# mfigura/Resilient-consensus-based-MARL

Measured on AMD Instinct MI355X. Metric: agent-steps/sec (whole RPBCAC training loop; + consensus-updates/sec), higher is better.
Workload: dtype f32 (matrix-core operands as 2 x f16 pieces: each fp32 operand to <= 1 ulp; the 20-unit layers run 3 of the 4 piece products)

## Files before the change

### include/rcmarl.h

```cpp
#ifndef RCMARL_H
#define RCMARL_H

#ifdef __cplusplus
extern "C" {
#endif

#define RCMARL_OK 0
#define RCMARL_ERR_ARG 1
#define RCMARL_ERR_LAUNCH 2
#define RCMARL_ERR_UNSUPPORTED 3

int rcmarl_abi_version(void);
int rcmarl_mb_job_layout(int what);
int rcmarl_fit_partial_size(int hid);
int rcmarl_actor_partial_size(int hid, int n_actions);
int rcmarl_rows_per_chunk(void);

int rcmarl_consensus_params(const float* msg, float* theta, const int* nbr, const int* coop, int S, int N,
                            int ldp, int P_hid, int d, int H, float* lo_dbg, float* hi_dbg, void* stream);
int rcmarl_consensus_params_circulant_supported(int N, int d, int H);
int rcmarl_consensus_params_circulant(const float* msg, float* theta, const int* coop, int S, int N, int ldp, int P_hid,
                                      int d, int H, float* lo_dbg, float* hi_dbg, void* stream);

typedef struct rcmarl_ragged_class {
// ... 15 lines not shown
                                float* adam_v, const int* mask, int S, int N, int B, int in_dim, int hid,
                                int ldp, int ldb, float alpha, float one_m_b1, float one_m_b2, float eps, void* stream);

int rcmarl_mid_fit(float* a1t, const float* theta, const float* y, float* partials, int S, int N, int B, int in_dim,
                   int hid, int ldp, int ldb, void* stream);
int rcmarl_lattice_f16_mode(void);
int rcmarl_lattice_set_f16_mode(int mode);
int rcmarl_lattice_forget(const void* buf);
int rcmarl_lattice_encode(const float* x, long x_seed_stride, const float* alpha, int S, int B, int in_dim, void* kp,
                          int kp_rt, int kp_kt, void* ktp, int ktp_rt, int ktp_kt, int* flag, void* stream);
int rcmarl_w1_split(const float* theta, const float* alpha, void* wp, int S, int N, int in_dim, int hid, int ldp,
                    int wp_rt, int wp_kt, void* stream);
int rcmarl_lattice_pack_dz(const float* dz, void* dzp, int S, int N, int B, int hid, int ldb, int dzp_rt, int dzp_kt,
                           void* stream);
int rcmarl_lattice_pack_dz_rowsum(const float* dz, void* dzp, float* sums, int sums_ld, int sums_off, int S, int N, int B, int hid,
                                  int ldb, int dzp_rt, int dzp_kt, void* stream);
int rcmarl_layer1_forward_lattice(const void* kp, int kp_rt, int kp_kt, const void* wp, int wp_rt, int wp_kt,
                                  const float* theta, float* a1t, int S, int N, int B, int in_dim, int hid, int ldp,
                                  int ldb, void* stream);
int rcmarl_layer1_backward_sgd_lattice(const void* ktp, int ktp_rt, int ktp_kt, const void* dzp, int dzp_rt, int dzp_kt,
                                       const float* alpha, float* theta, const int* mask, int S, int N, int B,
                                       int in_dim, int hid, int ldp, float lr, void* wp_out, int wp_rt, int wp_kt,
                                       void* stream);
int rcmarl_mid_fit_lattice(const float* a1t, const float* theta, const float* y, float* partials, void* dzp, int dzp_rt,
                           int dzp_kt, int S, int N, int B, int in_dim, int hid, int ldp, int ldb, int* ovf_flags, void* stream);


int rcmarl_shuffle_perms(const void* seeds, const int* calls, int n, int epochs, int B, int* perm, int S, void* stream);

int rcmarl_small_sgd(const float* partials, float* theta, const int* mask, float* loss_out, int S, int N,
                     int B, int in_dim, int hid, int ldp, float lr, void* stream);
int rcmarl_mid_value(const float* a1t, const float* theta, const float* r_applied, float gamma, float* out, int S,
                     int N, int B, int in_dim, int hid, int ldp, int ldb, void* stream);
int rcmarl_mid_value_f32(const float* a1t, const float* theta, const float* r_applied, float gamma, float* out, int S,
                         int N, int B, int in_dim, int hid, int ldp, int ldb, void* stream);

int rcmarl_consensus_head(const float* a1t, const float* theta, const float* msg, const int* nbr,
                          const int* coop, float* partials, float* agg_out, int S, int N, int B, int in_dim,
                          int hid, int ldp, int ldb, int d, int H, void* stream);
int rcmarl_consensus_head_ragged(const float* a1t, const float* theta, const float* msg, const int* nbr_off,
                                 const int* nbr_idx, const int* order, const rcmarl_ragged_class* classes, int n_classes,
                                 float* partials, float* agg_out, int S, int N, int B, int in_dim, int hid, int ldp, int ldb,
                                 void* stream);
int rcmarl_projection_residual(const float* a1t, const float* theta, const float* agg, const int* coop,
                               float* partials, int S, int N, int B, int in_dim, int hid, int ldp, int ldb,
                               void* stream);
// ... 167 lines not shown
```

### resilient-consensus-based-marl_amd/capi.py

```python
import ctypes as C
import os

c_f32p = C.c_void_p
c_i32p = C.c_void_p
c_u8p = C.c_void_p


class MbJob(C.Structure):
    _fields_ = [("x", C.c_void_p), ("x_seed_stride", C.c_long), ("theta", C.c_void_p), ("agents", C.c_void_p), ("n_adv", C.c_int),
                ("in_dim", C.c_int), ("ldp", C.c_int), ("reserved_", C.c_int), ("y", C.c_void_p), ("perm", C.c_void_p),
                ("loss_out", C.c_void_p), ("ovf_flags", C.c_void_p)]


class RaggedClass(C.Structure):
    _fields_ = [("d", C.c_int), ("H", C.c_int), ("first", C.c_int), ("count", C.c_int)]


c_f64p = C.c_void_p
c_stream = C.c_void_p

c_long = C.c_long
c_int = C.c_int
c_float = C.c_float

# ... 17 lines not shown
    "rcmarl_consensus_params_circulant": [c_f32p, c_f32p, c_u8p, c_int, c_int, c_int, c_int, c_int, c_int, c_f32p, c_f32p,
                                          c_stream],
    "rcmarl_ragged_class_layout": [c_int],
    "rcmarl_consensus_params_ragged": [c_f32p, c_f32p, c_i32p, c_i32p, c_i32p, C.c_void_p, c_int, c_int, c_int, c_int, c_int,
                                       c_f32p, c_f32p, c_stream],
    "rcmarl_consensus_head_ragged": [c_f32p, c_f32p, c_f32p, c_i32p, c_i32p, c_i32p, C.c_void_p, c_int, c_f32p, c_f32p, c_int,
                                     c_int, c_int, c_int, c_int, c_int, c_int, c_stream],
    "rcmarl_layer1_forward": [c_f32p, c_long, c_f32p, c_f32p, c_int, c_int, c_int, c_int, c_int, c_int, c_int,
                              c_stream],
    "rcmarl_layer1_backward_sgd": [c_f32p, c_long, c_f32p, c_f32p, c_u8p, c_int, c_int, c_int, c_int, c_int, c_int,
                                   c_int, c_float, c_stream],
    "rcmarl_layer1_backward_adam": [c_f32p, c_long, c_f32p, c_f32p, c_f32p, c_f32p, c_u8p, c_int, c_int, c_int, c_int,
                                    c_int, c_int, c_int, c_float, c_float, c_float, c_float, c_stream],
    "rcmarl_mid_fit": [c_f32p, c_f32p, c_f32p, c_f32p, c_int, c_int, c_int, c_int, c_int, c_int, c_int, c_stream],
    "rcmarl_lattice_encode": [c_f32p, c_long, c_f32p, c_int, c_int, c_int, c_u8p, c_int, c_int, c_u8p, c_int, c_int,
                              c_i32p, c_stream],
    "rcmarl_w1_split": [c_f32p, c_f32p, c_u8p, c_int, c_int, c_int, c_int, c_int, c_int, c_int, c_stream],
    "rcmarl_lattice_pack_dz": [c_f32p, c_u8p, c_int, c_int, c_int, c_int, c_int, c_int, c_int, c_stream],
    "rcmarl_lattice_pack_dz_rowsum": [c_f32p, c_u8p, c_f32p, c_int, c_int, c_int, c_int, c_int, c_int, c_int, c_int, c_int, c_stream],
    "rcmarl_layer1_forward_lattice": [c_u8p, c_int, c_int, c_u8p, c_int, c_int, c_f32p, c_f32p, c_int, c_int, c_int,
                                      c_int, c_int, c_int, c_int, c_stream],
    "rcmarl_layer1_backward_sgd_lattice": [c_u8p, c_int, c_int, c_u8p, c_int, c_int, c_f32p, c_f32p, c_u8p, c_int,
                                           c_int, c_int, c_int, c_int, c_int, c_float, c_u8p, c_int, c_int, c_stream],
    "rcmarl_mid_fit_lattice": [c_f32p, c_f32p, c_f32p, c_f32p, c_u8p, c_int, c_int, c_int, c_int, c_int, c_int, c_int,
                               c_int, c_int, c_i32p, c_stream],
    "rcmarl_shuffle_perms": [C.c_void_p, c_i32p, c_int, c_int, c_int, c_i32p, c_int, c_stream],
    "rcmarl_small_sgd": [c_f32p, c_f32p, c_u8p, c_f32p, c_int, c_int, c_int, c_int, c_int, c_int, c_float, c_stream],
    "rcmarl_mid_value": [c_f32p, c_f32p, c_f32p, c_float, c_f32p, c_int, c_int, c_int, c_int, c_int, c_int, c_int,
                         c_stream],
    "rcmarl_mid_value_f32": [c_f32p, c_f32p, c_f32p, c_float, c_f32p, c_int, c_int, c_int, c_int, c_int, c_int, c_int,
                             c_stream],
    "rcmarl_consensus_head": [c_f32p, c_f32p, c_f32p, c_i32p, c_u8p, c_f32p, c_f32p, c_int, c_int, c_int, c_int, c_int,
                              c_int, c_int, c_int, c_int, c_stream],
    "rcmarl_head_apply": [c_f32p, c_f32p, c_u8p, c_int, c_int, c_int, c_int, c_int, c_int, c_stream],
    "rcmarl_mid_actor": [c_f32p, c_f32p, c_f32p, c_f32p, c_f32p, c_int, c_int, c_int, c_int, c_int, c_int, c_int,
                         c_int, c_stream],
    "rcmarl_small_adam": [c_f32p, c_f32p, c_f32p, c_f32p, c_u8p, c_f32p, c_int, c_int, c_int, c_int, c_int, c_int,
                          c_int, c_float, c_float, c_float, c_float, c_stream],
    "rcmarl_team_reward": [c_f32p, c_long, c_u8p, c_int, c_f32p, c_int, c_int, c_int, c_int, c_stream],
    "rcmarl_projection_residual": [c_f32p, c_f32p, c_f32p, c_i32p, c_f32p, c_int, c_int, c_int, c_int, c_int, c_int,
                                   c_int, c_stream],
    "rcmarl_minibatch_fit": [c_f32p, c_long, c_f32p, c_i32p, c_int, c_f32p, c_i32p, c_int, c_int, c_int, c_int, c_int,
                             c_int, c_int, c_int, c_int, c_float, c_f32p, c_i32p, c_stream],
    "rcmarl_minibatch_actor": [c_f32p, c_long, c_f32p, c_f32p, c_f32p, c_i32p, c_int, c_f32p, c_f32p, c_i32p, c_int,
                               c_int, c_int, c_int, c_int, c_int, c_int, c_int, c_int, c_int, C.c_double, C.c_double,
                               C.c_double, C.c_double, c_int, c_f32p, c_stream],
# ... 58 lines not shown
    "rcmarl_policy_probs_wide": [c_f32p, c_f32p, c_f32p, c_int, c_int, c_int, c_int, c_int, c_int, c_stream],
    "rcmarl_rollout_step_wide": [c_f32p, c_i32p, c_i32p, c_f32p, C.c_void_p, c_int, c_int, c_f64p, c_f32p, c_f32p, c_f32p,
                                 c_f32p, c_f32p, c_long, c_long, c_i32p, c_f32p, c_f64p, C.c_double, c_int, c_int, c_float,
                                 c_int, c_int, c_int, c_int, c_int, c_i32p, c_stream],
    "rcmarl_rollout_wide_supported": [c_int],
    "rcmarl_policy_probs_episodes_wide": [c_f32p, c_f32p, c_f32p, c_int, c_int, c_int, c_int, c_int, c_int, c_int, c_stream],
    "rcmarl_rollout_step_episodes_wide": [c_f32p, c_i32p, c_i32p, c_f32p, C.c_void_p, c_int, c_int, c_f64p, c_f32p, c_f32p,
                                          c_f32p, c_f32p, c_f32p, c_long, c_long, c_int, c_i32p, c_f32p, c_f64p, C.c_double,
                                          c_int, c_int, c_float, c_int, c_int, c_int, c_int, c_int, c_int, c_int, c_stream],
    "rcmarl_dense_backward_adam": [c_f32p, c_long, c_long, c_int, c_int, c_f32p, c_f32p, c_f32p, c_f32p, c_int, c_i32p, c_int,
                                   c_int, c_int, c_int, c_int, c_int, c_int, c_float, c_float, c_float, c_float, c_stream],
    "rcmarl_wide_actor_head": [c_f32p, c_f32p, c_f32p, c_f32p, c_int, c_f32p, c_f32p, c_int, c_int, c_int, c_int, c_int, c_int,
                               c_int, c_int, c_stream],
    "rcmarl_wide_actor_small_adam": [c_f32p, c_f32p, c_f32p, c_f32p, c_f32p, c_f32p, c_f32p, c_i32p, c_f32p, c_int, c_int, c_int,
                                     c_int, c_int, c_int, c_int, c_int, c_float, c_float, c_float, c_float, c_stream],
    "rcmarl_copy3d": [c_f32p, c_long, c_long, c_f32p, c_long, c_long, c_int, c_int, c_int, c_i32p, c_stream],
}
UNCHECKED = {"rcmarl_abi_version", "rcmarl_mb_job_layout", "rcmarl_ragged_class_layout", "rcmarl_lattice_forget", "rcmarl_fit_partial_size", "rcmarl_lattice_set_f16_mode",  "rcmarl_actor_partial_size", "rcmarl_rows_per_chunk", "rcmarl_lattice_f16_mode",
             "rcmarl_wide_grad_size", "rcmarl_wide_rows_per_chunk", "rcmarl_wide_f16_mode", "rcmarl_wide_set_f16_mode",
             "rcmarl_consensus_params_circulant_supported", "rcmarl_pk_supported", "rcmarl_pk_parts",
             "rcmarl_rollout_wide_supported", "rcmarl_minibatch_fit_wide_supported",
             "rcmarl_minibatch_fit_wide2_supported"}

ERRORS = {1: "RCMARL_ERR_ARG (bad argument)", 2: "RCMARL_ERR_LAUNCH (HIP launch failed)",
          3: "RCMARL_ERR_UNSUPPORTED (shape outside the compiled kernels)"}


class RcmarlError(RuntimeError):
    pass


def _preload_hip_runtime():
    import torch
    cand = os.path.join(os.path.dirname(torch.__file__), "lib", "libamdhip64.so")
    try:
        C.CDLL(cand if os.path.exists(cand) else "libamdhip64.so.7", mode=C.RTLD_GLOBAL)
    except OSError as e:
        raise RcmarlError("cannot load the HIP runtime (libamdhip64): %s" % e)


class CLib:

    def __init__(self, path, needs_hip=True):
        if not os.path.exists(path):
            raise RcmarlError(
                "rcmarl HIP library not found at %s -- build it with `python -m rcmarl_amd.build` "
                "(hipcc --offload-arch=gfx950). There is no CPU fallback." % path)
        self.path = path
        if needs_hip:
            _preload_hip_runtime()
        self._dll = C.CDLL(path)
        for name, argtypes in SIGNATURES.items():
            fn = getattr(self._dll, name)
            fn.argtypes = argtypes
            fn.restype = C.c_int
            setattr(self, name, fn if name in UNCHECKED else self._checked(name, fn))

    @staticmethod
    def _checked(name, fn):
        def call(*args):
            rc = fn(*args)
            if rc != 0:
                raise RcmarlError("%s failed: %s" % (name, ERRORS.get(rc, rc)))
            return 0
        call.__name__ = name
        return call


_lib = None


def load():
    global _lib
    if _lib is None:
        from . import build
        _lib = CLib(build.lib_path())
    return _lib
```

### resilient-consensus-based-marl_amd/csrc/lattice_gemm.hip

```cpp
#include "rcmarl_lattice.h"
#include "rcmarl_lat_mainloop.h"
#include <type_traits>
#include <stdlib.h>

namespace {

__device__ __forceinline__ unsigned pack2(unsigned lo, unsigned hi) { return (lo & 0xffffu) | (hi << 16); }

__global__ __launch_bounds__(256) void k_lattice_encode(const float* __restrict__ x, long x_seed_stride,
                                                        const float* __restrict__ alpha, int B, int in_dim,
                                                        unsigned char* __restrict__ kp, int kp_rt, int kp_kt,
                                                        unsigned char* __restrict__ ktp, int ktp_rt, int ktp_kt,
                                                        int* __restrict__ flag, int kp_f16, int ktp_f16) {
  __shared__ unsigned short tileB[32][128 + 2], tileH[32][128 + 2];
  const int s = blockIdx.z, b0 = blockIdx.y * 32, c0 = blockIdx.x * 128;
  const int t = threadIdx.x;
  {
    const int cl = t & 127, c = c0 + cl;
    const float al = c < in_dim ? alpha[c] : 1.f;
    bool bad = false;
#pragma unroll 4
    for (int i = 0; i < 16; ++i) {
      const int bl = (t >> 7) + 2 * i, b = b0 + bl;
      float kq = 0.f;
// ... 272 lines not shown
    for (int nt = 0; nt < NT; ++nt) {
      const int n = bn * C::BN + wn * 32 * NT + 32 * nt + (lane & 31);
      if (n < B) {
        const unsigned lane_byte = ((unsigned)(4 * half) * (unsigned)ldb + (unsigned)n) * 4u;
#pragma unroll
        for (int mt = 0; mt < MT; ++mt) {
          const int m0 = bm * C::BM + wm * 32 * MT + 32 * mt;
          unsigned char* __restrict__ rowbase = reinterpret_cast<unsigned char*>(a1t_s + (long)m0 * ldb);
#pragma unroll
          for (int r = 0; r < 16; ++r) {
            const int dr = (r & 3) + 8 * (r >> 2);
            const float z = F16 ? fmaf(acc[mt][nt][r], RC_F16_W_UNSCALE, bv[mt][r]) : acc[mt][nt][r] + bv[mt][r];
            const float o = fmaxf(z, RC_LEAK * z);
            float* __restrict__ dst = reinterpret_cast<float*>(rowbase + (long)dr * ldb * 4 + lane_byte);
            if (FULL || m0 + dr + 4 * half < ncols) RC_NT_STORE(dst, o);
          }
        }
      }
    }
  };
  if (full_m) store_tile(std::true_type{}); else store_tile(std::false_type{});
}

template <bool W8, bool DZ16, bool WP16, bool M128 = false>
__global__ RC_LAT_OCC(W8 ? 512 : 256, W8 ? 4 : 2)
void k_lat_backward_sgd(const unsigned char* __restrict__ ktp, int ktp_rt, int ktp_kt, const unsigned char* __restrict__ dzp,
                        int dzp_rt, int dzp_kt, const float* __restrict__ alpha, float* __restrict__ theta,
                        const int* __restrict__ mask, int S, int N, int B, int in_dim, int ldp, float lr, int mtiles, int ntiles,
                        unsigned char* __restrict__ wp_out, int wp_rt, int wp_kt, int hid) {
  static_assert(!(W8 && M128), "the 128-row tile exists in the four-wavefront form");
  constexpr int PA = 1, PB = DZ16 ? 2 : 3, MT = W8 ? 2 : (M128 ? 2 : 4), NT = 2, WM = W8 ? 4 : 2, WN = 2;
  constexpr int WNP = WP16 ? 2 : 3;
  typedef LatCfg<PA, PB, MT, NT, WM, WN> C;
  RCMARL_DYN_SMEM(unsigned char, lds);
  int s, w;
  lat_decode(blockIdx.x, mtiles * ntiles, S, s, w);
  const int bm = w % mtiles, bn = w / mtiles;
  LatOperands op;
  op.a = ktp + (long)s * ktp_rt * ktp_kt * (PA * RC_PK_BLOCK); op.a_kt = ktp_kt; op.art0 = bm * C::ART;
  op.b = dzp + (long)s * dzp_rt * dzp_kt * (PB * RC_PK_BLOCK); op.b_kt = dzp_kt; op.brt0 = bn * C::BRT;
  rc_f32x16 acc[MT][NT];
  lat_mainloop<PA, PB, MT, NT, WM, WN, !W8, DZ16>(op, (B + 31) >> 5, lds, acc);
  const int ncols = N * hid;
  if (WP16) rc_f16_saturate();
  __syncthreads();
  float* al = reinterpret_cast<float*>(lds);
  if (threadIdx.x < C::BM) {
    const int k = bm * C::BM + threadIdx.x;
    al[threadIdx.x] = k < in_dim ? alpha[k] : 0.f;
  }
  __syncthreads();
  const int lane = threadIdx.x & 63, half = lane >> 5;
  const int wave = __builtin_amdgcn_readfirstlane((int)(threadIdx.x >> 6)), wm = wave / WN, wn = wave % WN;
  const bool full_k = (bm + 1) * C::BM <= in_dim;
#pragma unroll
  for (int nt = 0; nt < NT; ++nt) {
    const int cl = wn * 32 * NT + 32 * nt + (lane & 31);
    const int col = bn * C::BN + cl;
    const bool act = col < ncols;
    const int colc = act ? col : 0;
    const int ag = colc / hid, j = colc - ag * hid;
    const bool upd = act && (mask == nullptr || mask[ag]);
    const int k0 = bm * C::BM + wm * 32 * MT + 4 * half;
    float* th = theta + ((long)s * N + ag) * ldp + j + (long)k0 * hid;
    unsigned char* wrow = wp_out == nullptr ? nullptr
        : wp_out + (long)s * wp_rt * wp_kt * (WNP * RC_PK_BLOCK) + (long)(colc >> 7) * wp_kt * (WNP * RC_PK_BLOCK) + (colc & 127) * 64;
    const int sw = (colc >> 2) & 3;
    float wold[MT][16];
#pragma unroll
    for (int mt = 0; mt < MT; ++mt)
#pragma unroll
      for (int q = 0; q < 16; ++q) {
        const int dk = 32 * mt + 8 * (q >> 2) + (q & 3);
        wold[mt][q] = (act && (full_k || k0 + dk < in_dim)) ? th[(long)dk * hid] : 0.f;
      }
#pragma unroll
    for (int mt = 0; mt < MT; ++mt) {
      const int kt = bm * (C::BM / 32) + wm * MT + mt;
#pragma unroll
      for (int gp = 0; gp < 2; ++gp) {
        unsigned pc[2][WNP][2];
#pragma unroll
        for (int g1 = 0; g1 < 2; ++g1) {
          const int gq = 2 * gp + g1;
          const float4 a4 = *reinterpret_cast<const float4*>(al + wm * 32 * MT + 32 * mt + 8 * gq + 4 * half);
          const float av[4] = {a4.x, a4.y, a4.z, a4.w};
          float wn4[4];
#pragma unroll
          for (int e = 0; e < 4; ++e) {
            const int dk = 32 * mt + 8 * gq + e;
            float w = wold[mt][4 * gq + e];
            if (upd && (full_k || k0 + dk < in_dim)) {
              w = w - lr * (av[e] * acc[mt][nt][4 * gq + e]);
              th[(long)dk * hid] = w;
            }
            wn4[e] = w * av[e];
          }
          if constexpr (WP16) {
            rc_split2h_pair(wn4[0] * RC_F16_W_SCALE, wn4[1] * RC_F16_W_SCALE, pc[g1][0][0], pc[g1][1][0]);
            rc_split2h_pair(wn4[2] * RC_F16_W_SCALE, wn4[3] * RC_F16_W_SCALE, pc[g1][0][1], pc[g1][1][1]);
          } else {
            rc_split3_pair(wn4[0], wn4[1], pc[g1][0][0], pc[g1][1][0], pc[g1][2][0]);
            rc_split3_pair(wn4[2], wn4[3], pc[g1][0][1], pc[g1][1][1], pc[g1][2][1]);
          }
        }
        if (wp_out != nullptr && kt < wp_kt) {
#pragma unroll
          for (int p = 0; p < WNP; ++p)
#pragma unroll
            for (int dw = 0; dw < 2; ++dw) rc_swap_halves(pc[0][p][dw], pc[1][p][dw]);
          if (act) {
            unsigned char* q = wrow + (long)kt * (WNP * RC_PK_BLOCK) + (((2 * gp + half) ^ sw) << 4);
#pragma unroll
            for (int p = 0; p < WNP; ++p)
            {
              uint4 v;
              v.x = pc[0][p][0]; v.y = pc[0][p][1]; v.z = pc[1][p][0]; v.w = pc[1][p][1];
              st_u4(q + p * RC_PK_BLOCK, v);
            }
          }
        }
      }
    }
  }
}

int lat_env_int(const char* name, int dflt) { const char* e = getenv(name); return e ? atoi(e) : dflt; }
bool lat_w8(bool forward) { const char* e = getenv("RCMARL_LAT_W8"); return e ? atoi(e) != 0 : forward; }

template <bool W8, bool F16, bool PK = false>
int launch_forward(unsigned nblocks, void* stream, const unsigned char* wp, int wp_rt, int wp_kt, const unsigned char* kp, int kp_rt,
                   int kp_kt, const float* theta, float* a1t, int S, int N, int B, int in_dim, int ldp, int ldb, int mtiles,
                   int ntiles, int hid, const LatPkOut pk = LatPkOut{}) {
  const size_t smem = (size_t)2 * LatCfg<F16 ? 2 : 3, 1, 2, 4>::STAGE_BYTES;
  static const bool ok = rc_want_lds(k_lat_forward<W8, F16, PK>, smem);
  if (!ok) return RCMARL_ERR_LAUNCH;
  RCMARL_LAUNCH((k_lat_forward<W8, F16, PK>), dim3(nblocks), dim3(W8 ? 512 : 256), smem, stream, wp, wp_rt, wp_kt, kp, kp_rt, kp_kt,
                theta, a1t, S, N, B, in_dim, ldp, ldb, mtiles, ntiles, hid, pk);
  return rcmarl_check_launch();
}

template <bool W8, bool DZ16, bool WP16, bool M128 = false>
int launch_backward(unsigned nblocks, void* stream, const unsigned char* ktp, int ktp_rt, int ktp_kt, const unsigned char* dzp,
                    int dzp_rt, int dzp_kt, const float* alpha, float* theta, const int* mask, int S, int N, int B, int in_dim,
                    int ldp, float lr, int mtiles, int ntiles, unsigned char* wp_out, int wp_rt, int wp_kt, int hid) {
  const size_t smem = (size_t)2 * LatCfg<1, DZ16 ? 2 : 3, 4, 2>::STAGE_BYTES;
  static const bool ok = rc_want_lds(k_lat_backward_sgd<W8, DZ16, WP16, M128>, smem);
  if (!ok) return RCMARL_ERR_LAUNCH;
  RCMARL_LAUNCH((k_lat_backward_sgd<W8, DZ16, WP16, M128>), dim3(nblocks), dim3(W8 ? 512 : 256), smem, stream, ktp, ktp_rt, ktp_kt, dzp,
                dzp_rt, dzp_kt, alpha, theta, mask, S, N, B, in_dim, ldp, DZ16 ? lr * RC_F16_DZ_UNSCALE : lr, mtiles, ntiles,
                wp_out, wp_rt, wp_kt, hid);
  return rcmarl_check_launch();
}

}


RCMARL_EXPORT int rcmarl_lattice_encode(const float* x, long x_seed_stride, const float* alpha, int S, int B, int in_dim,
                                        void* kp, int kp_rt, int kp_kt, void* ktp, int ktp_rt, int ktp_kt, int* flag,
                                        void* stream) {
  if (!x || !alpha || !flag || S <= 0 || B <= 0 || in_dim <= 0 || (!kp && !ktp)) return RCMARL_ERR_ARG;
  const int b_pad = rc_ceil_div(B, 256) * 256;
  if (kp && (kp_rt * 128 < b_pad || kp_kt * 32 < in_dim)) return RCMARL_ERR_ARG;
  if (ktp && (ktp_rt * 128 < in_dim || ktp_kt * 32 < b_pad)) return RCMARL_ERR_ARG;
  int c_ext = in_dim;
  if (kp) c_ext = kp_kt * 32 > c_ext ? kp_kt * 32 : c_ext;
  if (ktp) c_ext = ktp_rt * 128 > c_ext ? ktp_rt * 128 : c_ext;
  const dim3 grid(rc_ceil_div(c_ext, 128), b_pad / 32, S), block(256);
  const int mode = rc_lat_f16_mode();
  rc_form_set(kp, mode & 1);
  rc_form_set(ktp, (mode >> 1) & 1);
  RCMARL_LAUNCH(k_lattice_encode, grid, block, 0, stream, x, x_seed_stride, alpha, B, in_dim, (unsigned char*)kp, kp_rt,
                kp_kt, (unsigned char*)ktp, ktp_rt, ktp_kt, flag, mode & 1, (mode >> 1) & 1);
  return rcmarl_check_launch();
}
// ... 68 lines not shown
}

RCMARL_EXPORT int rcmarl_layer1_forward_lattice_pk(const void* kp, int kp_rt, int kp_kt, const void* wp, int wp_rt, int wp_kt,
                                                   const float* theta, void* a1_bk, int bk_rt, void* a1_kb, int kb_kt,
                                                   unsigned* s1, int s1_ld, int* ovf_flag, int S, int N, int B, int in_dim, int hid,
                                                   int ldp, void* stream) {
  if (!kp || !wp || !theta || (!a1_bk && !a1_kb && !s1) || S <= 0 || N <= 0 || B <= 0 || in_dim <= 0 || hid <= 0 || (ldp & 63) ||
      ldp < in_dim * hid + hid)
    return RCMARL_ERR_ARG;
  if (hid & 127) return RCMARL_ERR_UNSUPPORTED;
  const int mtiles = N * hid / 128, ntiles = rc_ceil_div(B, 256), ktiles = rc_ceil_div(in_dim, 32);
  if (wp_rt < mtiles || kp_rt < 2 * ntiles || wp_kt < ktiles || kp_kt < ktiles) return RCMARL_ERR_ARG;
  if ((a1_bk && bk_rt < 2 * ntiles) || (a1_kb && kb_kt < 8 * ntiles) || (s1 && s1_ld < 8 * ntiles)) return RCMARL_ERR_ARG;
  if (!(rc_lat_f16_mode() & 1)) return RCMARL_ERR_UNSUPPORTED;
  if (!rc_form_ok(kp, true) || !rc_form_ok(wp, true)) return RCMARL_ERR_ARG;
  const unsigned nb = (unsigned)(S * mtiles * ntiles);
  LatPkOut pk;
  pk.a1_bk = (unsigned char*)a1_bk; pk.bk_rt = bk_rt; pk.a1_kb = (unsigned char*)a1_kb; pk.kb_kt = kb_kt; pk.s1 = s1; pk.s1_ld = s1_ld;
  pk.ovf = ovf_flag;
  return launch_forward<true, true, true>(nb, stream, (const unsigned char*)wp, wp_rt, wp_kt, (const unsigned char*)kp, kp_rt, kp_kt, theta,
                                          nullptr, S, N, B, in_dim, ldp, 64, mtiles, ntiles, hid, pk);
}

static int backward_sgd_lattice_impl(const void* ktp, int ktp_rt, int ktp_kt, const void* dzp, int dzp_rt,
                                                     int dzp_kt, const float* alpha, float* theta, const int* mask,
                                                     int S, int N, int B, int in_dim, int hid, int ldp, float lr,
                                                     void* wp_out, int wp_rt, int wp_kt, void* stream) {
  if (!ktp || !dzp || !alpha || !theta || S <= 0 || N <= 0 || B <= 0 || in_dim <= 0 || (ldp & 63) ||
      ldp < in_dim * hid + hid)
    return RCMARL_ERR_ARG;
  if (hid <= 0) return RCMARL_ERR_ARG;
  const bool w8 = lat_w8(false);
  const int m128_env = lat_env_int("RCMARL_LAT_M128", 1);
  const bool m128 = !w8 && ((in_dim <= 128 && m128_env != 0) || m128_env == 2);
  const int mtiles = m128 ? rc_ceil_div(in_dim, 128) : rc_ceil_div(in_dim, 256);
  const int ntiles = rc_ceil_div(N * hid, 128), ktiles = rc_ceil_div(B, 32);
  if (ktp_rt < (m128 ? mtiles : 2 * mtiles) || dzp_rt < ntiles || ktp_kt < ktiles || dzp_kt < ktiles) return RCMARL_ERR_ARG;
  if (wp_out && ((long)wp_rt * 128 < (long)ntiles * 128 || wp_kt < rc_ceil_div(in_dim, 32))) return RCMARL_ERR_ARG;
  const unsigned nb = (unsigned)(S * mtiles * ntiles);
  const int mode = rc_lat_f16_mode();
  if (!rc_form_ok(ktp, (mode >> 1) & 1) || !rc_form_ok(dzp, (mode >> 1) & 1)) return RCMARL_ERR_ARG;
  rc_form_set(wp_out, mode & 1);
#define RC_BWD(W8, DZ16, WP16)                                                                                              \
  launch_backward<W8, DZ16, WP16>(nb, stream, (const unsigned char*)ktp, ktp_rt, ktp_kt, (const unsigned char*)dzp, dzp_rt, \
                                  dzp_kt, alpha, theta, mask, S, N, B, in_dim, ldp, lr, mtiles, ntiles,                     \
                                  (unsigned char*)wp_out, wp_rt, wp_kt, hid)
  if (m128) {
#define RC_BWD128(DZ16, WP16)                                                                                                  \
  launch_backward<false, DZ16, WP16, true>(nb, stream, (const unsigned char*)ktp, ktp_rt, ktp_kt, (const unsigned char*)dzp,  \
                                           dzp_rt, dzp_kt, alpha, theta, mask, S, N, B, in_dim, ldp, lr, mtiles, ntiles,       \
                                           (unsigned char*)wp_out, wp_rt, wp_kt, hid)
    switch (mode) {
      case 0: return RC_BWD128(false, false);
      case 1: return RC_BWD128(false, true);
      case 2: return RC_BWD128(true, false);
      default: return RC_BWD128(true, true);
    }
#undef RC_BWD128
  }
  switch (mode * 2 + (w8 ? 1 : 0)) {
    case 0: return RC_BWD(false, false, false);
    case 1: return RC_BWD(true, false, false);
    case 2: return RC_BWD(false, false, true);
    case 3: return RC_BWD(true, false, true);
    case 4: return RC_BWD(false, true, false);
    case 5: return RC_BWD(true, true, false);
    case 6: return RC_BWD(false, true, true);
    default: return RC_BWD(true, true, true);
  }
#undef RC_BWD
}

RCMARL_EXPORT int rcmarl_layer1_backward_sgd_lattice(const void* ktp, int ktp_rt, int ktp_kt, const void* dzp, int dzp_rt,
                                                     int dzp_kt, const float* alpha, float* theta, const int* mask,
                                                     int S, int N, int B, int in_dim, int hid, int ldp, float lr,
                                                     void* wp_out, int wp_rt, int wp_kt, void* stream) {
  return backward_sgd_lattice_impl(ktp, ktp_rt, ktp_kt, dzp, dzp_rt, dzp_kt, alpha, theta, mask, S, N, B, in_dim, hid, ldp, lr, wp_out,
                                   wp_rt, wp_kt, stream);
}
```

### resilient-consensus-based-marl_amd/engine.py

```python
import contextlib
import gc
import math
import os
import time

import numpy as np
import torch

from . import capi
from . import lattice as LT

HID = 20
COOP, FAULTY, GREEDY, MALICIOUS = "Cooperative", "Faulty", "Greedy", "Malicious"


def pad64(n):
    return (int(n) + 63) // 64 * 64


def net_numel(in_dim, out_dim, hid=HID):
    return in_dim * hid + hid + hid * hid + hid + hid * out_dim + out_dim


def net_shapes(in_dim, out_dim, hid=HID):
    return [(in_dim, hid), (hid,), (hid, hid), (hid,), (hid, out_dim), (out_dim,)]


def flatten_params(params):
    return np.concatenate([np.asarray(p, dtype=np.float32).ravel() for p in params])


def unflatten_params(vec, in_dim, out_dim, hid=HID):
    out, o = [], 0
    for sh in net_shapes(in_dim, out_dim, hid):
        n = int(np.prod(sh))
        out.append(np.array(vec[o:o + n], dtype=np.float32).reshape(sh))
        o += n
    return out


class EngineConfig:

    def __init__(self, n_agents, agent_label, in_nodes, H=0, gamma=0.9, slow_lr=0.002, fast_lr=0.01, n_actions=5,
                 n_states=2, max_ep_len=20, n_ep_fixed=50, n_epochs=10, buffer_size=2000, common_reward=False,
                 nrow=5, ncol=5, n_seeds=1, rng_mode="device", mu=0.1, scaling=True, randomize_state=True,
                 local_fit_steps=5, lattice="auto", critic_hid=HID, actor_hid=HID, tr_hid=HID, adv_wide2="auto"):
        self.n_agents, self.agent_label = int(n_agents), list(agent_label)
        self.in_nodes = [list(map(int, row)) for row in in_nodes]
        self.gamma, self.slow_lr, self.fast_lr = float(gamma), float(slow_lr), float(fast_lr)
        self.n_actions, self.n_states = int(n_actions), int(n_states)
        self.max_ep_len, self.n_ep_fixed, self.n_epochs = int(max_ep_len), int(n_ep_fixed), int(n_epochs)
        self.buffer_size, self.common_reward = int(buffer_size), bool(common_reward)
        self.nrow, self.ncol, self.n_seeds = int(nrow), int(ncol), int(n_seeds)
        self.rng_mode, self.mu, self.scaling, self.randomize_state = rng_mode, float(mu), bool(scaling), bool(randomize_state)
        self.local_fit_steps = int(local_fit_steps)
        self.lattice = lattice
        self.critic_hid = int(critic_hid)
        self.actor_hid = int(actor_hid)
        self.tr_hid = int(tr_hid)
        if not any(adv_wide2 is v for v in (True, False)) and adv_wide2 != "auto":
            raise ValueError("adv_wide2 must be 'auto', True or False")
        self.adv_wide2 = adv_wide2
        assert len(self.agent_label) == self.n_agents and len(self.in_nodes) == self.n_agents
        if np.ndim(H) == 0:
            self.H_per_agent = [int(H)] * self.n_agents
        else:
            self.H_per_agent = [int(h) for h in H]
            if len(self.H_per_agent) != self.n_agents:
                raise ValueError("H must be an int or one int per agent (got %d for %d agents)" % (len(self.H_per_agent), self.n_agents))
        self.degrees = [len(row) for row in self.in_nodes]
        for i, row in enumerate(self.in_nodes):
            if not row or row[0] != i:
                raise ValueError("in_nodes[i][0] must be i (own value first, agents/resilient_CAC_agents.py:49)")
            if any(j < 0 or j >= self.n_agents for j in row):
                raise ValueError("in_nodes[%d] names an agent outside 0..%d" % (i, self.n_agents - 1))
            if self.agent_label[i] == COOP and (self.H_per_agent[i] < 0 or len(row) < 2 * self.H_per_agent[i] + 1):
                raise ValueError("need d >= 2H+1 (agent %d: d = %d, H = %d)" % (i, len(row), self.H_per_agent[i]))
        self.regular = len(set(self.degrees)) == 1 and len(set(self.H_per_agent)) == 1
        self.H = self.H_per_agent[0] if self.regular else max([h for h, l in zip(self.H_per_agent, self.agent_label) if l == COOP],
                                                               default=max(self.H_per_agent))
        if self.n_states != 2 or self.n_actions != 5:
            raise ValueError("the grid-world has 2 state dims and 5 actions per agent")
        if rng_mode not in ("device", "numpy"):
            raise ValueError("rng_mode must be 'device' or 'numpy'")
        for lab in self.agent_label:
# ... 528 lines not shown
        env = os.environ.get("RCMARL_LATTICE")
        if env is not None:
            want = env not in ("0", "false", "False", "")
        if want == "auto":
            want = self.N >= 16
        self.lat_enabled = bool(want)
        self.lat_active = False
        if not self.lat_enabled:
            return
        u8 = lambda rk, pieces: torch.zeros(self.S * LT.Geometry.nbytes(rk, pieces), dtype=torch.uint8, device=self.dev)
        self.lat_geom = {"s": LT.Geometry(self.N, self.in_c, self.cap, self.hid["critic"]),
                         "sa": LT.Geometry(self.N, self.in_r, self.cap, self.hid["tr"])}
        self.lat_geom["ns"] = self.lat_geom["s"]
        self.lat_kp = {k: u8(self.lat_geom[k].kp, 1) for k in ("s", "ns", "sa")}
        self.lat_ktp = {k: u8(self.lat_geom[k].ktp, 1) for k in ("s", "sa")}
        self.lat_wp_f = {"sa": u8(self.lat_geom["sa"].wp, 3), "s": u8(self.lat_geom["s"].wp, 3)}
        self.lat_dzp_f = {"sa": u8(self.lat_geom["sa"].dzp, 3), "s": u8(self.lat_geom["s"].dzp, 3)}
        self.lat_wp_f["ns"] = self.lat_wp_f["s"]
        f32 = dict(dtype=torch.float32, device=self.dev)
        self.lat_alpha = {"s": torch.tensor(LT.column_alpha(self.N, 2, c.nrow, c.ncol, c.scaling), **f32),
                          "sa": torch.tensor(LT.column_alpha(self.N, 3, c.nrow, c.ncol, c.scaling), **f32)}
        self.lat_alpha["ns"] = self.lat_alpha["s"]
        self.lat_flag = torch.zeros(1, dtype=torch.int32, device=self.dev)
        self.lat_geom_term = LT.Geometry(self.N, self.in_c, max(1, -(-self.cap // max(c.max_ep_len, 1))), self.hid["critic"])
        self.lat_kp_term = u8(self.lat_geom_term.kp, 1)
        self.lat_flag_term = torch.zeros(1, dtype=torch.int32, device=self.dev)

    def __del__(self):
        try:
            forget = getattr(self.lib, "rcmarl_lattice_forget", None)
            if forget is None or not getattr(self, "lat_enabled", False):
                return
            for d in (self.lat_kp, self.lat_ktp, self.lat_wp_f, self.lat_dzp_f):
                for t in d.values():
                    forget(t.data_ptr())
            forget(self.lat_kp_term.data_ptr())
        except Exception:
            pass

    def _lattice_encode(self, B):
        self.lat_active = False
        if not self.lat_enabled:
            return
        L = self.lib
        self.lat_flag.zero_()
        for k in ("s", "ns", "sa"):
# ... 344 lines not shown
            return
        a1 = self.a1net[net]
        ptr, stride = self._x(xkey)
        lat = self._lattice_ok(xkey, B, 0) and xkey in self.lat_ktp
        g = self.lat_geom[xkey] if lat else None
        dzp, wp = (self.lat_dzp_f[xkey], self.lat_wp_f[xkey]) if lat else (None, None)
        partials = self.partials if partials is None else partials
        wp_fresh = False
        for step in range(self.cfg.local_fit_steps):
            if not (step == 0 and self.a1_cached[net]):
                self._layer1(xkey, msg, net, B, buf=a1, wp_fresh=wp_fresh)
            if lat:
                L.rcmarl_mid_fit_lattice(a1.data_ptr(), msg.data_ptr(), y.data_ptr(), partials.data_ptr(),
                                         dzp.data_ptr(), g.dzp[0], g.dzp[1], S, N, B, self.in_dim[net], HID,
                                         self.ldp[net], self.ldb, self.ovf_flags(("mid", net), S * N + 1).data_ptr(), self.stream)
            else:
                L.rcmarl_mid_fit(a1.data_ptr(), msg.data_ptr(), y.data_ptr(), partials.data_ptr(), S, N, B,
                                 self.in_dim[net], HID, self.ldp[net], self.ldb, self.stream)
            L.rcmarl_small_sgd(partials.data_ptr(), msg.data_ptr(), mask.data_ptr(),
                               self.loss[net].data_ptr() if step == 0 else None, S, N, B, self.in_dim[net], HID,
                               self.ldp[net], self.cfg.fast_lr, self.stream)
            if lat:
                last = step == self.cfg.local_fit_steps - 1
                L.rcmarl_layer1_backward_sgd_lattice(self.lat_ktp[xkey].data_ptr(), g.ktp[0], g.ktp[1],
                                                     dzp.data_ptr(), g.dzp[0], g.dzp[1],
                                                     self.lat_alpha[xkey].data_ptr(), msg.data_ptr(), mask.data_ptr(), S, N,
                                                     B, self.in_dim[net], HID, self.ldp[net], self.cfg.fast_lr,
                                                     None if last else wp.data_ptr(), g.wp[0], g.wp[1], self.stream)
                wp_fresh = True
            else:
                L.rcmarl_layer1_backward_sgd(ptr, stride, a1.data_ptr(), msg.data_ptr(), mask.data_ptr(), S, N, B,
                                             self.in_dim[net], HID, self.ldp[net], self.ldb, self.cfg.fast_lr, self.stream)
        self.a1_cached[net] = False

    def ovf_flags(self, key, n):
        d = self.__dict__.setdefault("_ovf_flags", {})
        t = d.get(key)
        if t is None or t.numel() < n:
            t = d[key] = torch.zeros(int(n), dtype=torch.int32, device=self.dev)
        return t

    def _fit_as_chains(self, net, mask):
        if self.hid[net] != HID or self.in_dim[net] > 20 or self.lat_active or mask is not self.coop or self.n_coop == 0:
            return False
        if self.dev.type != "cuda" and os.environ.get("RCMARL_FIT_CHAINS") != "1":
            return False
        e = os.environ.get("RCMARL_FIT_CHAINS")
        if e is not None:
            return e not in ("0", "false")
        return self.S * self.n_coop >= 1024

# ... 492 lines not shown
```

### resilient-consensus-based-marl_amd/timing.py

```python
import collections

import torch

from . import capi


def _gemm_flops(a, first):
    S, N, B, in_dim, hid = a[first:first + 5]
    return 2.0 * S * N * hid * B * in_dim, 0.0


_LIB = None


def lattice_pieces(bit, lib=None):
    lib = lib or _LIB or capi.load()
    return 2 if int(lib.rcmarl_lattice_f16_mode()) & bit else 3


WORK = {
    "rcmarl_layer1_forward": lambda a: _gemm_flops(a, 4),
    "rcmarl_layer1_backward_sgd": lambda a: _gemm_flops(a, 5),
    "rcmarl_layer1_backward_adam": lambda a: _gemm_flops(a, 7),
    "rcmarl_consensus_params": lambda a: (0.0, 8.0 * a[4] * a[5] * a[7]),
    "rcmarl_consensus_params_circulant": lambda a: (0.0, 8.0 * a[3] * a[4] * a[6]),
    "rcmarl_mid_fit": lambda a: (a[4] * a[5] * a[6] * (8.0 * a[8] ** 2 + 12.0 * a[8]), 8.0 * a[4] * a[5] * a[6] * a[8]),
    "rcmarl_layer1_forward_lattice": lambda a: _gemm_flops(a, 8),
    "rcmarl_layer1_backward_sgd_lattice": lambda a: _gemm_flops(a, 9),
    "rcmarl_mid_fit_lattice": lambda a: (a[7] * a[8] * a[9] * (8.0 * a[11] ** 2 + 12.0 * a[11]),
                                         (4.0 + 2.0 * lattice_pieces(2)) * a[7] * a[8] * a[9] * a[11]),
    "rcmarl_w1_split": lambda a: (0.0, (4.0 + 2.0 * lattice_pieces(1)) * a[3] * a[4] * a[5] * a[6]),
    "rcmarl_minibatch_fit": lambda a: (6.0 * a[7] * a[4] * a[15] * a[9] * (a[10] * a[11] + a[11] * a[11] + a[11]), 0.0),
    "rcmarl_minibatch_fit_multi": lambda a: (sum(6.0 * a[2] * j.n_adv * a[8] * a[4] * (j.in_dim * a[5] + a[5] * a[5] + a[5])
                                                 for j in list(a[0])[:a[1]]) if hasattr(a[0], "__len__") else 0.0, 0.0),
    "rcmarl_dense_forward": lambda a: (2.0 * a[9] * a[10] * a[11] * a[12] * a[13], 0.0),
    "rcmarl_dense_backward_data": lambda a: (2.0 * a[5] * a[6] * a[7] * a[8] * a[9], 0.0),
    "rcmarl_dense_backward_sgd": lambda a: (2.0 * a[9] * a[10] * a[11] * a[12] * a[13], 0.0),
    "rcmarl_layer1_forward_lattice_pk": lambda a: _gemm_flops(a, 14),
    "rcmarl_pk_forward2": lambda a: (2.0 * a[11] * a[12] * a[13] * a[15] * a[15], 0.0),
    "rcmarl_pk_backward_data": lambda a: (2.0 * a[12] * a[13] * a[14] * a[15] * a[15], 0.0),
    "rcmarl_pk_backward_w2": lambda a: (2.0 * a[9] * a[10] * a[11] * a[13] * a[13], 0.0),
}


class TimedLib:
    def __init__(self, lib):
        global _LIB
        self._lib = _LIB = lib
        self.enabled = False
        self._events = collections.defaultdict(list)
        self.work = {}
        for name in capi.SIGNATURES:
            fn = getattr(lib, name)
            setattr(self, name, fn if name in capi.UNCHECKED else self._wrap(name, fn))

    def _wrap(self, name, fn):
        def call(*args):
            if not self.enabled:
                return fn(*args)
            e0, e1 = torch.cuda.Event(enable_timing=True), torch.cuda.Event(enable_timing=True)
            e0.record()
            r = fn(*args)
            e1.record()
            self._events[name].append((e0, e1))
            if name in WORK:
                f, b = WORK[name](args)
                pf, pb = self.work.get(name, (0.0, 0.0))
                self.work[name] = (pf + f, pb + b)
            return r
        return call

    def reset(self):
        self._events.clear()
        self.work = {}

    def summary(self):
        out = {}
# ... 5 lines not shown
```

Before: 21.78 million.

## Keep layer-1 weights in a lane-tiled scratch buffer across local fit steps

```diff
diff --git a/include/rcmarl.h b/include/rcmarl.h
--- a/include/rcmarl.h
+++ b/include/rcmarl.h
@@ -61,6 +61,11 @@
                                        const float* alpha, float* theta, const int* mask, int S, int N, int B,
                                        int in_dim, int hid, int ldp, float lr, void* wp_out, int wp_rt, int wp_kt,
                                        void* stream);
+int rcmarl_layer1_backward_sgd_lattice_tiled(const void* ktp, int ktp_rt, int ktp_kt, const void* dzp, int dzp_rt, int dzp_kt,
+                                             const float* alpha, float* theta, const int* mask, int S, int N, int B,
+                                             int in_dim, int hid, int ldp, float lr, void* wp_out, int wp_rt, int wp_kt,
+                                             float* w_tiled, long w_tiled_bytes, int src_tiled, int dst_tiled, void* stream);
+long rcmarl_lattice_w1_tiled_bytes(int S, int N, int in_dim, int hid);
 int rcmarl_mid_fit_lattice(const float* a1t, const float* theta, const float* y, float* partials, void* dzp, int dzp_rt,
                            int dzp_kt, int S, int N, int B, int in_dim, int hid, int ldp, int ldb, int* ovf_flags, void* stream);
 
diff --git a/resilient-consensus-based-marl_amd/capi.py b/resilient-consensus-based-marl_amd/capi.py
--- a/resilient-consensus-based-marl_amd/capi.py
+++ b/resilient-consensus-based-marl_amd/capi.py
@@ -63,6 +63,9 @@
                                       c_int, c_int, c_int, c_int, c_stream],
     "rcmarl_layer1_backward_sgd_lattice": [c_u8p, c_int, c_int, c_u8p, c_int, c_int, c_f32p, c_f32p, c_u8p, c_int,
                                            c_int, c_int, c_int, c_int, c_int, c_float, c_u8p, c_int, c_int, c_stream],
+    "rcmarl_layer1_backward_sgd_lattice_tiled": [c_u8p, c_int, c_int, c_u8p, c_int, c_int, c_f32p, c_f32p, c_u8p, c_int,
+                                                 c_int, c_int, c_int, c_int, c_int, c_float, c_u8p, c_int, c_int, c_f32p, c_long,
+                                                 c_int, c_int, c_stream],
     "rcmarl_mid_fit_lattice": [c_f32p, c_f32p, c_f32p, c_f32p, c_u8p, c_int, c_int, c_int, c_int, c_int, c_int, c_int,
                                c_int, c_int, c_i32p, c_stream],
     "rcmarl_shuffle_perms": [C.c_void_p, c_i32p, c_int, c_int, c_int, c_i32p, c_int, c_stream],
@@ -167,6 +170,10 @@
              "rcmarl_rollout_wide_supported", "rcmarl_minibatch_fit_wide_supported",
              "rcmarl_minibatch_fit_wide2_supported"}
 
+LONG_QUERIES = {
+    "rcmarl_lattice_w1_tiled_bytes": [c_int, c_int, c_int, c_int],
+}
+
 ERRORS = {1: "RCMARL_ERR_ARG (bad argument)", 2: "RCMARL_ERR_LAUNCH (HIP launch failed)",
           3: "RCMARL_ERR_UNSUPPORTED (shape outside the compiled kernels)"}
 
@@ -200,6 +207,11 @@
             fn.argtypes = argtypes
             fn.restype = C.c_int
             setattr(self, name, fn if name in UNCHECKED else self._checked(name, fn))
+        for name, argtypes in LONG_QUERIES.items():
+            fn = getattr(self._dll, name)
+            fn.argtypes = argtypes
+            fn.restype = C.c_long
+            setattr(self, name, fn)
 
     @staticmethod
     def _checked(name, fn):
diff --git a/resilient-consensus-based-marl_amd/csrc/lattice_gemm.hip b/resilient-consensus-based-marl_amd/csrc/lattice_gemm.hip
--- a/resilient-consensus-based-marl_amd/csrc/lattice_gemm.hip
+++ b/resilient-consensus-based-marl_amd/csrc/lattice_gemm.hip
@@ -318,13 +318,14 @@
   if (full_m) store_tile(std::true_type{}); else store_tile(std::false_type{});
 }
 
-template <bool W8, bool DZ16, bool WP16, bool M128 = false>
+template <bool W8, bool DZ16, bool WP16, bool M128 = false, int ROLE = 0>
 __global__ RC_LAT_OCC(W8 ? 512 : 256, W8 ? 4 : 2)
 void k_lat_backward_sgd(const unsigned char* __restrict__ ktp, int ktp_rt, int ktp_kt, const unsigned char* __restrict__ dzp,
                         int dzp_rt, int dzp_kt, const float* __restrict__ alpha, float* __restrict__ theta,
                         const int* __restrict__ mask, int S, int N, int B, int in_dim, int ldp, float lr, int mtiles, int ntiles,
-                        unsigned char* __restrict__ wp_out, int wp_rt, int wp_kt, int hid) {
+                        unsigned char* __restrict__ wp_out, int wp_rt, int wp_kt, int hid, float* __restrict__ w_tiled) {
   static_assert(!(W8 && M128), "the 128-row tile exists in the four-wavefront form");
+  constexpr bool SRC_T = (ROLE & 1) != 0, DST_T = (ROLE & 2) != 0;
   constexpr int PA = 1, PB = DZ16 ? 2 : 3, MT = W8 ? 2 : (M128 ? 2 : 4), NT = 2, WM = W8 ? 4 : 2, WN = 2;
   constexpr int WNP = WP16 ? 2 : 3;
   typedef LatCfg<PA, PB, MT, NT, WM, WN> C;
@@ -359,6 +360,11 @@
     const bool upd = act && (mask == nullptr || mask[ag]);
     const int k0 = bm * C::BM + wm * 32 * MT + 4 * half;
     float* th = theta + ((long)s * N + ag) * ldp + j + (long)k0 * hid;
+    const long tl_mt = (long)(ntiles * 4) * 1024;
+    float* tl = nullptr;
+    (void)tl_mt; (void)tl; (void)th;
+    if constexpr (SRC_T || DST_T)
+      tl = w_tiled + (((long)s * (((in_dim + 255) >> 8) * 8) + (bm * (C::BM / 32) + wm * MT)) * (ntiles * 4) + (bn * (C::BN / 32) + wn * NT + nt)) * 1024 + lane;
     unsigned char* wrow = wp_out == nullptr ? nullptr
         : wp_out + (long)s * wp_rt * wp_kt * (WNP * RC_PK_BLOCK) + (long)(colc >> 7) * wp_kt * (WNP * RC_PK_BLOCK) + (colc & 127) * 64;
     const int sw = (colc >> 2) & 3;
@@ -368,7 +374,8 @@
 #pragma unroll
       for (int q = 0; q < 16; ++q) {
         const int dk = 32 * mt + 8 * (q >> 2) + (q & 3);
-        wold[mt][q] = (act && (full_k || k0 + dk < in_dim)) ? th[(long)dk * hid] : 0.f;
+        if constexpr (SRC_T) wold[mt][q] = tl[mt * tl_mt + q * 64];
+        else wold[mt][q] = (act && (full_k || k0 + dk < in_dim)) ? th[(long)dk * hid] : 0.f;
       }
 #pragma unroll
     for (int mt = 0; mt < MT; ++mt) {
@@ -388,8 +395,9 @@
             float w = wold[mt][4 * gq + e];
             if (upd && (full_k || k0 + dk < in_dim)) {
               w = w - lr * (av[e] * acc[mt][nt][4 * gq + e]);
-              th[(long)dk * hid] = w;
+              if constexpr (!DST_T) th[(long)dk * hid] = w;
             }
+            if constexpr (DST_T) tl[mt * tl_mt + (4 * gq + e) * 64] = w;
             wn4[e] = w * av[e];
           }
           if constexpr (WP16) {
@@ -436,17 +444,28 @@
   return rcmarl_check_launch();
 }
 
-template <bool W8, bool DZ16, bool WP16, bool M128 = false>
-int launch_backward(unsigned nblocks, void* stream, const unsigned char* ktp, int ktp_rt, int ktp_kt, const unsigned char* dzp,
-                    int dzp_rt, int dzp_kt, const float* alpha, float* theta, const int* mask, int S, int N, int B, int in_dim,
-                    int ldp, float lr, int mtiles, int ntiles, unsigned char* wp_out, int wp_rt, int wp_kt, int hid) {
+template <bool W8, bool DZ16, bool WP16, bool M128, int ROLE>
+int launch_backward_role(unsigned nblocks, void* stream, const unsigned char* ktp, int ktp_rt, int ktp_kt, const unsigned char* dzp,
+                         int dzp_rt, int dzp_kt, const float* alpha, float* theta, const int* mask, int S, int N, int B, int in_dim,
+                         int ldp, float lr, int mtiles, int ntiles, unsigned char* wp_out, int wp_rt, int wp_kt, int hid,
+                         float* w_tiled) {
   const size_t smem = (size_t)2 * LatCfg<1, DZ16 ? 2 : 3, 4, 2>::STAGE_BYTES;
-  static const bool ok = rc_want_lds(k_lat_backward_sgd<W8, DZ16, WP16, M128>, smem);
+  static const bool ok = rc_want_lds(k_lat_backward_sgd<W8, DZ16, WP16, M128, ROLE>, smem);
   if (!ok) return RCMARL_ERR_LAUNCH;
-  RCMARL_LAUNCH((k_lat_backward_sgd<W8, DZ16, WP16, M128>), dim3(nblocks), dim3(W8 ? 512 : 256), smem, stream, ktp, ktp_rt, ktp_kt, dzp,
-                dzp_rt, dzp_kt, alpha, theta, mask, S, N, B, in_dim, ldp, DZ16 ? lr * RC_F16_DZ_UNSCALE : lr, mtiles, ntiles,
-                wp_out, wp_rt, wp_kt, hid);
+  RCMARL_LAUNCH((k_lat_backward_sgd<W8, DZ16, WP16, M128, ROLE>), dim3(nblocks), dim3(W8 ? 512 : 256), smem, stream, ktp, ktp_rt, ktp_kt,
+                dzp, dzp_rt, dzp_kt, alpha, theta, mask, S, N, B, in_dim, ldp, DZ16 ? lr * RC_F16_DZ_UNSCALE : lr, mtiles, ntiles,
+                wp_out, wp_rt, wp_kt, hid, w_tiled);
   return rcmarl_check_launch();
+}
+
+template <bool W8, bool DZ16, bool WP16, bool M128 = false, typename... A>
+int launch_backward(int role, A... a) {
+  switch (role) {
+    case 0: return launch_backward_role<W8, DZ16, WP16, M128, 0>(a...);
+    case 1: return launch_backward_role<W8, DZ16, WP16, M128, 1>(a...);
+    case 2: return launch_backward_role<W8, DZ16, WP16, M128, 2>(a...);
+    default: return launch_backward_role<W8, DZ16, WP16, M128, 3>(a...);
+  }
 }
 
 }
@@ -561,14 +580,24 @@
                                           nullptr, S, N, B, in_dim, ldp, 64, mtiles, ntiles, hid, pk);
 }
 
+static long lat_w1_tiled_bytes(int S, int N, int in_dim, int hid) {
+  if (S <= 0 || N <= 0 || in_dim <= 0 || hid <= 0) return -1;
+  const long kt = (long)rc_ceil_div(in_dim, 256) * 8, ct = ((long)N * hid + 127) / 128 * 4;
+  return (long)S * kt * ct * 4096;
+}
+
 static int backward_sgd_lattice_impl(const void* ktp, int ktp_rt, int ktp_kt, const void* dzp, int dzp_rt,
                                                      int dzp_kt, const float* alpha, float* theta, const int* mask,
                                                      int S, int N, int B, int in_dim, int hid, int ldp, float lr,
-                                                     void* wp_out, int wp_rt, int wp_kt, void* stream) {
+                                                     void* wp_out, int wp_rt, int wp_kt, void* stream,
+                                                     float* w_tiled = nullptr, long w_tiled_bytes = 0, int role = 0) {
   if (!ktp || !dzp || !alpha || !theta || S <= 0 || N <= 0 || B <= 0 || in_dim <= 0 || (ldp & 63) ||
       ldp < in_dim * hid + hid)
     return RCMARL_ERR_ARG;
   if (hid <= 0) return RCMARL_ERR_ARG;
+  if (role != 0 && (!w_tiled || (reinterpret_cast<uintptr_t>(w_tiled) & 3) || w_tiled_bytes < lat_w1_tiled_bytes(S, N, in_dim, hid)))
+    return RCMARL_ERR_ARG;
+  if ((role & 2) && !wp_out) return RCMARL_ERR_ARG;
   const bool w8 = lat_w8(false);
   const int m128_env = lat_env_int("RCMARL_LAT_M128", 1);
   const bool m128 = !w8 && ((in_dim <= 128 && m128_env != 0) || m128_env == 2);
@@ -581,14 +610,14 @@
   if (!rc_form_ok(ktp, (mode >> 1) & 1) || !rc_form_ok(dzp, (mode >> 1) & 1)) return RCMARL_ERR_ARG;
   rc_form_set(wp_out, mode & 1);
 #define RC_BWD(W8, DZ16, WP16)                                                                                              \
-  launch_backward<W8, DZ16, WP16>(nb, stream, (const unsigned char*)ktp, ktp_rt, ktp_kt, (const unsigned char*)dzp, dzp_rt, \
-                                  dzp_kt, alpha, theta, mask, S, N, B, in_dim, ldp, lr, mtiles, ntiles,                     \
-                                  (unsigned char*)wp_out, wp_rt, wp_kt, hid)
+  launch_backward<W8, DZ16, WP16>(role, nb, stream, (const unsigned char*)ktp, ktp_rt, ktp_kt, (const unsigned char*)dzp, dzp_rt, \
+                                  dzp_kt, alpha, theta, mask, S, N, B, in_dim, ldp, lr, mtiles, ntiles,                           \
+                                  (unsigned char*)wp_out, wp_rt, wp_kt, hid, w_tiled)
   if (m128) {
 #define RC_BWD128(DZ16, WP16)                                                                                                  \
-  launch_backward<false, DZ16, WP16, true>(nb, stream, (const unsigned char*)ktp, ktp_rt, ktp_kt, (const unsigned char*)dzp,  \
-                                           dzp_rt, dzp_kt, alpha, theta, mask, S, N, B, in_dim, ldp, lr, mtiles, ntiles,       \
-                                           (unsigned char*)wp_out, wp_rt, wp_kt, hid)
+  launch_backward<false, DZ16, WP16, true>(role, nb, stream, (const unsigned char*)ktp, ktp_rt, ktp_kt, (const unsigned char*)dzp,  \
+                                           dzp_rt, dzp_kt, alpha, theta, mask, S, N, B, in_dim, ldp, lr, mtiles, ntiles,             \
+                                           (unsigned char*)wp_out, wp_rt, wp_kt, hid, w_tiled)
     switch (mode) {
       case 0: return RC_BWD128(false, false);
       case 1: return RC_BWD128(false, true);
@@ -617,3 +646,14 @@
   return backward_sgd_lattice_impl(ktp, ktp_rt, ktp_kt, dzp, dzp_rt, dzp_kt, alpha, theta, mask, S, N, B, in_dim, hid, ldp, lr, wp_out,
                                    wp_rt, wp_kt, stream);
 }
+
+RCMARL_EXPORT long rcmarl_lattice_w1_tiled_bytes(int S, int N, int in_dim, int hid) { return lat_w1_tiled_bytes(S, N, in_dim, hid); }
+
+RCMARL_EXPORT int rcmarl_layer1_backward_sgd_lattice_tiled(const void* ktp, int ktp_rt, int ktp_kt, const void* dzp, int dzp_rt,
+                                                           int dzp_kt, const float* alpha, float* theta, const int* mask,
+                                                           int S, int N, int B, int in_dim, int hid, int ldp, float lr,
+                                                           void* wp_out, int wp_rt, int wp_kt, float* w_tiled, long w_tiled_bytes,
+                                                           int src_tiled, int dst_tiled, void* stream) {
+  return backward_sgd_lattice_impl(ktp, ktp_rt, ktp_kt, dzp, dzp_rt, dzp_kt, alpha, theta, mask, S, N, B, in_dim, hid, ldp, lr, wp_out,
+                                   wp_rt, wp_kt, stream, w_tiled, w_tiled_bytes, (src_tiled ? 1 : 0) | (dst_tiled ? 2 : 0));
+}
diff --git a/resilient-consensus-based-marl_amd/engine.py b/resilient-consensus-based-marl_amd/engine.py
--- a/resilient-consensus-based-marl_amd/engine.py
+++ b/resilient-consensus-based-marl_amd/engine.py
@@ -12,6 +12,7 @@
 
 HID = 20
 COOP, FAULTY, GREEDY, MALICIOUS = "Cooperative", "Faulty", "Greedy", "Malicious"
+W1_TILED_AUTO = True
 
 
 def pad64(n):
@@ -44,7 +45,8 @@
     def __init__(self, n_agents, agent_label, in_nodes, H=0, gamma=0.9, slow_lr=0.002, fast_lr=0.01, n_actions=5,
                  n_states=2, max_ep_len=20, n_ep_fixed=50, n_epochs=10, buffer_size=2000, common_reward=False,
                  nrow=5, ncol=5, n_seeds=1, rng_mode="device", mu=0.1, scaling=True, randomize_state=True,
-                 local_fit_steps=5, lattice="auto", critic_hid=HID, actor_hid=HID, tr_hid=HID, adv_wide2="auto"):
+                 local_fit_steps=5, lattice="auto", critic_hid=HID, actor_hid=HID, tr_hid=HID, adv_wide2="auto",
+                 w1_tiled="auto"):
         self.n_agents, self.agent_label = int(n_agents), list(agent_label)
         self.in_nodes = [list(map(int, row)) for row in in_nodes]
         self.gamma, self.slow_lr, self.fast_lr = float(gamma), float(slow_lr), float(fast_lr)
@@ -61,6 +63,9 @@
         if not any(adv_wide2 is v for v in (True, False)) and adv_wide2 != "auto":
             raise ValueError("adv_wide2 must be 'auto', True or False")
         self.adv_wide2 = adv_wide2
+        if not any(w1_tiled is v for v in (True, False)) and w1_tiled != "auto":
+            raise ValueError("w1_tiled must be 'auto', True or False")
+        self.w1_tiled = w1_tiled
         assert len(self.agent_label) == self.n_agents and len(self.in_nodes) == self.n_agents
         if np.ndim(H) == 0:
             self.H_per_agent = [int(H)] * self.n_agents
@@ -635,6 +640,12 @@
                           "sa": torch.tensor(LT.column_alpha(self.N, 3, c.nrow, c.ncol, c.scaling), **f32)}
         self.lat_alpha["ns"] = self.lat_alpha["s"]
         self.lat_flag = torch.zeros(1, dtype=torch.int32, device=self.dev)
+        want = W1_TILED_AUTO if c.w1_tiled == "auto" else c.w1_tiled
+        fams = [net for net in ("critic", "tr") if self.hid[net] == HID]
+        self.lat_w1_tiled = None
+        if want and c.local_fit_steps >= 2 and fams:
+            nbytes = max(int(self.lib.rcmarl_lattice_w1_tiled_bytes(self.S, self.N, self.in_dim[net], HID)) for net in fams)
+            self.lat_w1_tiled = torch.zeros(nbytes // 4, **f32)
         self.lat_geom_term = LT.Geometry(self.N, self.in_c, max(1, -(-self.cap // max(c.max_ep_len, 1))), self.hid["critic"])
         self.lat_kp_term = u8(self.lat_geom_term.kp, 1)
         self.lat_flag_term = torch.zeros(1, dtype=torch.int32, device=self.dev)
@@ -1025,11 +1036,15 @@
                                self.ldp[net], self.cfg.fast_lr, self.stream)
             if lat:
                 last = step == self.cfg.local_fit_steps - 1
-                L.rcmarl_layer1_backward_sgd_lattice(self.lat_ktp[xkey].data_ptr(), g.ktp[0], g.ktp[1],
-                                                     dzp.data_ptr(), g.dzp[0], g.dzp[1],
-                                                     self.lat_alpha[xkey].data_ptr(), msg.data_ptr(), mask.data_ptr(), S, N,
-                                                     B, self.in_dim[net], HID, self.ldp[net], self.cfg.fast_lr,
-                                                     None if last else wp.data_ptr(), g.wp[0], g.wp[1], self.stream)
+                args = (self.lat_ktp[xkey].data_ptr(), g.ktp[0], g.ktp[1], dzp.data_ptr(), g.dzp[0], g.dzp[1],
+                        self.lat_alpha[xkey].data_ptr(), msg.data_ptr(), mask.data_ptr(), S, N, B, self.in_dim[net], HID,
+                        self.ldp[net], self.cfg.fast_lr, None if last else wp.data_ptr(), g.wp[0], g.wp[1])
+                wt = self.lat_w1_tiled
+                if wt is not None and self.cfg.local_fit_steps >= 2:
+                    L.rcmarl_layer1_backward_sgd_lattice_tiled(*args, wt.data_ptr(), 4 * wt.numel(), int(step > 0), int(not last),
+                                                               self.stream)
+                else:
+                    L.rcmarl_layer1_backward_sgd_lattice(*args, self.stream)
                 wp_fresh = True
             else:
                 L.rcmarl_layer1_backward_sgd(ptr, stride, a1.data_ptr(), msg.data_ptr(), mask.data_ptr(), S, N, B,
diff --git a/resilient-consensus-based-marl_amd/timing.py b/resilient-consensus-based-marl_amd/timing.py
--- a/resilient-consensus-based-marl_amd/timing.py
+++ b/resilient-consensus-based-marl_amd/timing.py
@@ -27,6 +27,7 @@
     "rcmarl_mid_fit": lambda a: (a[4] * a[5] * a[6] * (8.0 * a[8] ** 2 + 12.0 * a[8]), 8.0 * a[4] * a[5] * a[6] * a[8]),
     "rcmarl_layer1_forward_lattice": lambda a: _gemm_flops(a, 8),
     "rcmarl_layer1_backward_sgd_lattice": lambda a: _gemm_flops(a, 9),
+    "rcmarl_layer1_backward_sgd_lattice_tiled": lambda a: _gemm_flops(a, 9),
     "rcmarl_mid_fit_lattice": lambda a: (a[7] * a[8] * a[9] * (8.0 * a[11] ** 2 + 12.0 * a[11]),
                                          (4.0 + 2.0 * lattice_pieces(2)) * a[7] * a[8] * a[9] * a[11]),
     "rcmarl_w1_split": lambda a: (0.0, (4.0 + 2.0 * lattice_pieces(1)) * a[3] * a[4] * a[5] * a[6]),
@@ -53,6 +54,8 @@
         for name in capi.SIGNATURES:
             fn = getattr(lib, name)
             setattr(self, name, fn if name in capi.UNCHECKED else self._wrap(name, fn))
+        for name in capi.LONG_QUERIES:
+            setattr(self, name, getattr(lib, name))
 
     def _wrap(self, name, fn):
         def call(*args):
```

Result: faster. 22.08 million (median of 6 runs) (+1.3%).
